# EBI-Metagenomics/deciphon

Hardware: AMD Instinct MI355X
Metric: GCUPS (Viterbi DP cell updates/sec) (higher is better)
Workload: dtype f32

## Files before the change

deciphon_amd/csrc/viterbi_body.h:

```cpp
#pragma once
#include "dcp_types.h"

#ifndef DCP_FN
#error "include a lane_ops_*.h before viterbi_body.h"
#endif

#define DCP_INF (__builtin_inff())

#define DCP_SL(P, t) (((P) + 5 - (t)) % 5)

#ifndef DCP_LAZY_POSITIONS
#define DCP_LAZY_POSITIONS 6
#endif
constexpr int dcp_lazy_turns(int Q) { return Q >= DCP_LAZY_POSITIONS ? 1 : (DCP_LAZY_POSITIONS + Q - 1) / Q; }

#ifndef DCP_SHAPE_POLICY
#define DCP_SHAPE_POLICY(Q, W) ((W) == 1 ? ((Q) > 8 ? 7 : (Q) == 8 ? 2 : 0) : ((Q) >= 8 ? 6 : 0))
#endif
#ifndef DCP_COST_POLICY
#define DCP_COST_POLICY(Q, W) (DCP_SHAPE_POLICY(Q, W) | ((W) == 1 && ((Q) == 4 || (Q) == 5) ? 1 : 0))
#endif
template <int Q, int W, bool STORE = false, int POLICY = DCP_SHAPE_POLICY(Q, W)> struct CostWave
{
  static constexpr int TURNS = dcp_lazy_turns(Q);
  static constexpr bool LATE_FETCH = (POLICY & 1) != 0;
  static constexpr bool STASH = (POLICY & 6) != 0;
  static constexpr bool STASH6 = (POLICY & 4) != 0;
  static constexpr bool CHUNKED = STASH6 && W == 1;
  static constexpr int SLOTS = STASH6 ? 8 : 4;
  Group<W> g;
  float *__restrict__ tab_cells = nullptr;
  float *__restrict__ tab_sp = nullptr;
  int tabKp = 0;
  float *__restrict__ ckpt_out = nullptr;
  float const *__restrict__ ckpt_in = nullptr;
  int ckpt_every = 0;
  int row_base = 0;

  DCP_FN void save_ring(float *__restrict__ to)
  {
#pragma unroll
    for (int s = 0; s < 5; ++s)
    {
      store_q<Q>(to + (size_t)s * tabKp, g.lane, Mpre[s]);
      store_q<Q>(to + (size_t)(5 + s) * tabKp, g.lane, Ipre[s]);
      store_lane(to + (size_t)10 * tabKp + s * 64 * W, g.lane, Spre[s]);
    }
    store_lane(to + (size_t)10 * tabKp + 5 * 64 * W, g.lane, X);
  }
  DCP_FN void load_ring(float const *__restrict__ from)
  {
#pragma unroll
    for (int s = 0; s < 5; ++s)
    {
      load_q<Q>(from + (size_t)s * tabKp, g.lane, Mpre[s]);
      load_q<Q>(from + (size_t)(5 + s) * tabKp, g.lane, Ipre[s]);
      Spre[s] = load_lane(from + (size_t)10 * tabKp + s * 64 * W, g.lane);
    }
    X = load_lane(from + (size_t)10 * tabKp + 5 * 64 * W, g.lane);
  }
  lf BM[Q], MM[Q], MI[Q], MD[Q], IM[Q], II[Q], DM[Q], DD[Q];
  lf Mpre[5][Q], Ipre[5][Q], Spre[5];
  lf em[5][Q];
  lf sa, sb;
  lf X;
  lf NBv, EBv, JBv;
  lf shM, shI, shD;
  float nil[5], bgv[5];
  float ET, CT, RR;
  float E;
  RowSrc rows;
  lu voff;
  uint32_t stride_bytes;
#ifdef DCP_COST_ORDER
  static constexpr bool ORDERED = !STORE && Q >= 5;
  lu voffc[ORDERED ? DcpRowChunks<Q>::N : 1];
#endif
  DcpCodeRow const *__restrict__ codes;

  DcpCodeRow cr;

  DCP_FN void fetch(int l_after, int L)
  {
#pragma unroll
    for (int t = 0; t < 5; ++t)
    {
      uint32_t const off = cr.c[t] * stride_bytes;
#ifdef DCP_COST_ORDER
      if constexpr (ORDERED)
      {
        load_row_hdr(rows, off, nil[t], bgv[t]);
        load_row_chunks<Q>(rows, voffc, off, em[t]);
        continue;
      }
#endif
      load_row_hdr(rows, off, nil[t], bgv[t]);
      load_row_q<Q>(rows, voff, off, em[t]);
    }
    cr = codes[l_after <= L ? l_after : L];
  }

  DCP_FN void init(float const *__restrict__ pool, DcpProfileDev const &pf, DcpCodeRow const *__restrict__ code_rows,
                   float const *__restrict__ xt)
  {
#ifndef DCP_WAVE_PRIO
#define DCP_WAVE_PRIO(Q, W) ((W) > 1 || (Q) >= 6 ? 3 : (Q) >= 4 ? 2 : (Q) == 3 ? 1 : 0)
#endif
    wave_priority<DCP_WAVE_PRIO(Q, W)>();
    g.init();
    lu const lane = g.lane;
    int const Kp = pf.Kp;
    stride_bytes = (uint32_t)(Kp + DCP_ROW_HDR) * 4u;
    int64_t rows_off = pf.rows_off;
#ifdef DCP_COST_ORDER
    if constexpr (ORDERED)
    {
      bool const copy = pf.cost_rows_off != 0 && pf.cost_shape == DCP_COST_SHAPE(Q, W);
      if (copy)
      {
        rows_off = pf.cost_rows_off;
        stride_bytes = 4u * (uint32_t)(DCP_COST_ORDER_HDR + 64 * Q * W);
      }
      row_chunk_offsets<Q, W>(lane, copy, voffc);
    }
#endif
    rows = rowsrc_make(pool + rows_off, (uint32_t)DCP_TABLE_SIZE * stride_bytes);
    voff = row_lane_offset<Q>(lane);
    codes = code_rows;
    float const *__restrict__ trans = pool + pf.trans_off;
    load_q<Q>(trans + DCP_BM * Kp, lane, BM);
    load_q<Q>(trans + DCP_MM * Kp, lane, MM);
    load_q<Q>(trans + DCP_MI * Kp, lane, MI);
    load_q<Q>(trans + DCP_MD * Kp, lane, MD);
    load_q<Q>(trans + DCP_IM * Kp, lane, IM);
    load_q<Q>(trans + DCP_II * Kp, lane, II);
    load_q<Q>(trans + DCP_DM * Kp, lane, DM);
    load_q<Q>(trans + DCP_DD * Kp, lane, DD);
    NBv = lf_pin(xt[DCP_NB]);
    EBv = lf_pin(xt[DCP_EB]);
    JBv = lf_pin(xt[DCP_JB]);
    shM = shI = shD = lf_splat(DCP_INF);
    g.put_tdd(DD);
    if constexpr (STASH)
    {
      g.template stash_q<Q, SLOTS>(0, MD);
      g.template stash_q<Q, SLOTS>(1, DD);
      g.template stash_q<Q, SLOTS>(2, II);
      g.template stash_q<Q, SLOTS>(3, MI);
      if constexpr (STASH6)
      {
        g.template stash_q<Q, SLOTS>(4, IM);
        g.template stash_q<Q, SLOTS>(5, DM);
        g.template stash_q<Q, SLOTS>(6, BM);
        g.template stash_q<Q, SLOTS>(7, MM);
      }
    }
    ET = xt[DCP_ET];
    CT = xt[DCP_CT];
    RR = xt[DCP_RR];
    float const SN = xt[DCP_SN], SB = xt[DCP_SB];
    lm const l0 = lequ(lane, lu_splat(0)), l1 = lequ(lane, lu_splat(1));
    lm const l2 = lequ(lane, lu_splat(2)), l3 = lequ(lane, lu_splat(3));
    lf const inf = lf_splat(DCP_INF);
    sa = lsel(l1, lf_splat(xt[DCP_EJ]), lsel(l2, lf_splat(xt[DCP_EC]), inf));
    sb = lsel(l0, lf_splat(xt[DCP_NN]),
              lsel(l1, lf_splat(xt[DCP_JJ]), lsel(l2, lf_splat(xt[DCP_CC]), lsel(l3, lf_splat(RR), inf))));
#pragma unroll
    for (int s = 0; s < 5; ++s)
    {
      Spre[s] = inf;
#pragma unroll
      for (int q = 0; q < Q; ++q)
      {
        Mpre[s][q] = inf;
        Ipre[s][q] = inf;
      }
    }
#pragma unroll
    for (int q = 0; q < Q; ++q) Mpre[0][q] = lf_splat(SB) + BM[q];
    Spre[0] = lsel(l0, lf_splat(0.0f + SN), lsel(l3, lf_splat(-RR + RR), inf));
    X = lsel(l3, lf_splat(-RR), inf);
    E = DCP_INF;
    tabKp = Kp;
    if (ckpt_in)
      load_ring(ckpt_in);
    else if (STORE)
      store_row0(SB);
  }

  template <int P> DCP_FN void row(int l, int L)
  {
    lf M[Q], I[Q];
#pragma unroll
    for (int q = 0; q < Q; ++q)
    {
      M[q] = lmin3(lmin3(Mpre[DCP_SL(P, 5)][q] + em[4][q], Mpre[DCP_SL(P, 4)][q] + em[3][q],
                         Mpre[DCP_SL(P, 3)][q] + em[2][q]),
                   Mpre[DCP_SL(P, 2)][q] + em[1][q], Mpre[DCP_SL(P, 1)][q] + em[0][q]);
      I[q] = lmin3(lmin3(Ipre[DCP_SL(P, 5)][q] + bgv[4], Ipre[DCP_SL(P, 4)][q] + bgv[3],
                         Ipre[DCP_SL(P, 3)][q] + bgv[2]),
                   Ipre[DCP_SL(P, 2)][q] + bgv[1], Ipre[DCP_SL(P, 1)][q] + bgv[0]);
    }
    X = lmin3(lmin3(Spre[DCP_SL(P, 5)] + nil[4], Spre[DCP_SL(P, 4)] + nil[3], Spre[DCP_SL(P, 3)] + nil[2]),
              Spre[DCP_SL(P, 2)] + nil[1], Spre[DCP_SL(P, 1)] + nil[0]);

    if constexpr (!LATE_FETCH)
      if (l < L) fetch(l + 2, L);

    lf m = M[0];
#pragma unroll
    for (int q = 1; q < Q; ++q) m = lmin(m, M[q]);
    lf D[Q];
    lf Msh0, Ish0, Dsh0, B;
    float N, J;
    if constexpr (STASH)
    {
      g.template unstash_q<Q, SLOTS>(0, MD);
      g.template unstash_q<Q, SLOTS>(1, DD);
    }
    if constexpr (W == 1)
    {
      Msh0 = lane_shift_up_keep(M[Q - 1], shM);
      Ish0 = lane_shift_up_keep(I[Q - 1], shI);
      E = wave_min(m);
      N = read_lane(X, 0);
      J = read_lane(X, 1);
      B = lmin3(N + NBv, E + EBv, J + JBv);

      D[0] = Msh0 + MD[0];
#pragma unroll
      for (int q = 1; q < Q; ++q) D[q] = lmin(M[q - 1] + MD[q], D[q - 1] + DD[q]);
      Dsh0 = lane_shift_up_keep(D[Q - 1], shD);
      lf x = Dsh0 + DD[0];
#pragma unroll
      for (int turn = 0; turn < TURNS; ++turn)
      {
        D[0] = lmin(D[0], x);
#pragma unroll
        for (int q = 1; q < Q; ++q) D[q] = lmin(D[q], D[q - 1] + DD[q]);
        Dsh0 = lane_shift_up_keep(D[Q - 1], shD);
        x = Dsh0 + DD[0];
      }
      while (wave_any(llt(x, D[0])))
      {
        D[0] = lmin(D[0], x);
#pragma unroll
        for (int q = 1; q < Q; ++q) D[q] = lmin(D[q], D[q - 1] + DD[q]);
        Dsh0 = lane_shift_up_keep(D[Q - 1], shD);
        x = Dsh0 + DD[0];
      }
    }
    else
    {
      int const par = l & 1;
      lf const inf = lf_splat(DCP_INF);
      lf x, Dsh;
      lm better;
      D[0] = g.seg_shift_up(M[Q - 1], inf) + MD[0];
#pragma unroll
      for (int q = 1; q < Q; ++q) D[q] = lmin(M[q - 1] + MD[q], D[q - 1] + DD[q]);
      Dsh = g.seg_shift_up(D[Q - 1], inf);
      x = Dsh + DD[0];
      better = llt(x, D[0]);
      while (g.seg_any(better))
      {
        D[0] = lmin(D[0], x);
#pragma unroll
        for (int q = 1; q < Q; ++q) D[q] = lmin(D[q], D[q - 1] + DD[q]);
        Dsh = g.seg_shift_up(D[Q - 1], inf);
        x = Dsh + DD[0];
        better = llt(x, D[0]);
      }
      g.put_rec(par, M[Q - 1], I[Q - 1], D[Q - 1], m);
      g.put_lanes4(GS_X0 + par, X);
      g.sync();
      lf Mp, Ip, Dp;
      bool could;
      g.get_prev(par, Mp, Ip, Dp);
      g.get_e_could(par, E, could);
      g.get_nj(GS_X0 + par, X, N, J);
      Msh0 = g.seg_shift_up(M[Q - 1], Mp);
      Ish0 = g.seg_shift_up(I[Q - 1], Ip);
      B = lmin3(N + NBv, E + EBv, J + JBv);
      if (!could)
      {
        D[0] = lsel(g.seg_first(), lmin(Mp + MD[0], Dp + DD[0]), D[0]);
#pragma unroll
        for (int q = 1; q < Q; ++q) D[q] = lmin(D[q], D[q - 1] + DD[q]);
        Dsh0 = g.seg_shift_up(D[Q - 1], Dp);
        x = Dsh0 + DD[0];
        better = llt(x, D[0]);
        while (g.seg_any(better))
        {
          D[0] = lmin(D[0], x);
#pragma unroll
          for (int q = 1; q < Q; ++q) D[q] = lmin(D[q], D[q - 1] + DD[q]);
          Dsh0 = g.seg_shift_up(D[Q - 1], Dp);
          x = Dsh0 + DD[0];
          better = llt(x, D[0]);
        }
      }
      else
      {
        g.note_fallback();
        D[0] = Msh0 + MD[0];
#pragma unroll
        for (int q = 1; q < Q; ++q) D[q] = lmin(M[q - 1] + MD[q], D[q - 1] + DD[q]);
        g.put_last(GS_D, D[Q - 1]);
        g.sync();
        Dsh0 = g.get_shift(GS_D, D[Q - 1], DCP_INF);
        x = Dsh0 + DD[0];
        better = llt(x, D[0]);
        g.put_any(GS_F, better);
        g.sync();
        while (g.get_any(GS_F, better))
        {
          D[0] = lmin(D[0], x);
#pragma unroll
          for (int q = 1; q < Q; ++q) D[q] = lmin(D[q], D[q - 1] + DD[q]);
          g.put_last(GS_D, D[Q - 1]);
          g.sync();
          Dsh0 = g.get_shift(GS_D, D[Q - 1], DCP_INF);
          x = Dsh0 + DD[0];
          better = llt(x, D[0]);
          g.put_any(GS_F, better);
          g.sync();
        }
      }
    }

    if constexpr (LATE_FETCH)
    {
      sched_fence();
      if (l < L) fetch(l + 2, L);
      sched_fence();
    }
    if constexpr (CHUNKED)
    {
      constexpr int N = DcpStashChunk<Q>::N;
#pragma unroll
      for (int j = 0; j < Q / N; ++j)
      {
        lf bm[N], mm[N], im[N], dm[N], ii[N], mi[N];
        g.template unstash_chunk<Q, SLOTS>(2, j, ii);
        g.template unstash_chunk<Q, SLOTS>(3, j, mi);
        g.template unstash_chunk<Q, SLOTS>(4, j, im);
        g.template unstash_chunk<Q, SLOTS>(5, j, dm);
        g.template unstash_chunk<Q, SLOTS>(6, j, bm);
        g.template unstash_chunk<Q, SLOTS>(7, j, mm);
#pragma unroll
        for (int i = 0; i < N; ++i)
        {
          int const q = N * j + i;
          lf const Ml = q ? M[q ? q - 1 : 0] : Msh0;
          lf const Il = q ? I[q ? q - 1 : 0] : Ish0;
          lf const Dl = q ? D[q ? q - 1 : 0] : Dsh0;
          Mpre[P][q] = lmin3(B + bm[i], Ml + mm[i], lmin(Il + im[i], Dl + dm[i]));
          Ipre[P][q] = lmin(I[q] + ii[i], M[q] + mi[i]);
        }
        sched_fence();
      }
    }
    else if constexpr (STASH)
    {
      g.template unstash_q<Q, SLOTS>(2, II);
      g.template unstash_q<Q, SLOTS>(3, MI);
      if constexpr (STASH6)
      {
        g.template unstash_q<Q, SLOTS>(4, IM);
        g.template unstash_q<Q, SLOTS>(5, DM);
        g.template unstash_q<Q, SLOTS>(6, BM);
        g.template unstash_q<Q, SLOTS>(7, MM);
      }
    }
    if constexpr (!CHUNKED)
    {
#pragma unroll
      for (int q = 0; q < Q; ++q)
      {
        lf const Ml = q ? M[q ? q - 1 : 0] : Msh0;
        lf const Il = q ? I[q ? q - 1 : 0] : Ish0;
        lf const Dl = q ? D[q ? q - 1 : 0] : Dsh0;
        Mpre[P][q] = lmin3(B + BM[q], Ml + MM[q], lmin(Il + IM[q], Dl + DM[q]));
        Ipre[P][q] = lmin(I[q] + II[q], M[q] + MI[q]);
      }
    }
    Spre[P] = lmin(lf_splat(E) + sa, X + sb);
    if (STORE)
    {
      float *row = tab_cells + (size_t)(l - row_base) * 3 * (size_t)tabKp;
      store_q<Q>(row, g.lane, M);
      store_q<Q>(row + tabKp, g.lane, I);
      store_q<Q>(row + 2 * tabKp, g.lane, D);
      float const C = g.get_lane(GS_X0 + (l & 1), X, 2);
      store_sp_lane0(tab_sp + (size_t)(l - row_base) * DCP_SP_STRIDE, g.lane, lf_splat(N), B, lf_splat(J), lf_splat(E),
                     lf_splat(C));
    }
  }

  DCP_FN void store_row0(float SB)
  {
    lf inf[Q];
#pragma unroll
    for (int q = 0; q < Q; ++q) inf[q] = lf_splat(DCP_INF);
    store_q<Q>(tab_cells, g.lane, inf);
    store_q<Q>(tab_cells + tabKp, g.lane, inf);
    store_q<Q>(tab_cells + 2 * tabKp, g.lane, inf);
    lf const i = lf_splat(DCP_INF);
    store_sp_lane0(tab_sp, g.lane, i, lf_splat(SB), i, i, i);
  }

  DCP_FN void run(int L, float *out, int Lend = -1)
  {
    if (Lend < 0 || Lend > L) Lend = L;
    int l = row_base + 1;
    if (l <= Lend)
    {
      cr = codes[l];
      fetch(l + 1, Lend);
    }
    for (; l + 4 <= Lend; l += 5)
    {
      row<1>(l, Lend);
      row<2>(l + 1, Lend);
      row<3>(l + 2, Lend);
      row<4>(l + 3, Lend);
      row<0>(l + 4, Lend);
      if (ckpt_every > 0 && (l + 4) % ckpt_every == 0 && l + 4 + 5 < L)
        save_ring(ckpt_out + (size_t)((l + 4) / ckpt_every - 1) * (size_t)dcp_ckpt_floats(tabKp, W));
    }
    if (l <= Lend) row<1>(l++, Lend);
    if (l <= Lend) row<2>(l++, Lend);
    if (l <= Lend) row<3>(l++, Lend);
    if (l <= Lend) row<4>(l++, Lend);
    if (Lend < L) return;
    g.sync();
    g.put_lanes4(GS_X, X);
    g.sync();
    float const C = g.get_lane(GS_X, X, 2);
    float const R = g.get_lane(GS_X, X, 3);
    float const T = L > 0 ? __builtin_fminf(E + ET, C + CT) : DCP_INF;
    store_f32_lane0(out + 0, g.lane, R);
    store_f32_lane0(out + 1, g.lane, T);
  }
};

template <int Q, int W, bool STORE = false> struct StripWave
{
  Group<W> g;
  float *__restrict__ tab_cells = nullptr;
  float *__restrict__ tab_sp = nullptr;
  float *__restrict__ ring = nullptr;
  float const *__restrict__ trans = nullptr;
  int Kp = 0, S = 0;
  lf Spre[5];
  lf sa, sb, X;
  float Bz[5];
  float NB, EB, JB, ET, CT, RR, E;
  RowSrc rows;
  lu voff;
  uint32_t stride_bytes;
  DcpCodeRow const *__restrict__ codes;
  int tick = 0;
  float *__restrict__ ckpt_out = nullptr;
  float const *__restrict__ ckpt_in = nullptr;
  int ckpt_every = 0;
  int row_base = 0;

  enum { KS = 64 * Q * W };

  DCP_FN void save_ring(float *__restrict__ to)
  {
    for (int s = 0; s < S; ++s)
      for (int z = 0; z < 10; ++z)
      {
        lf v[Q];
        load_q<Q>(ring + (size_t)z * Kp + (size_t)s * KS, g.lane, v);
        store_q<Q>(to + (size_t)z * Kp + (size_t)s * KS, g.lane, v);
      }
    float *sp = to + (size_t)10 * Kp;
#pragma unroll
    for (int z = 0; z < 5; ++z)
    {
      store_lane(sp + z * 64 * W, g.lane, Spre[z]);
      store_f32_lane0(sp + DCP_CKPT_SP * 64 * W + z, g.lane, Bz[z]);
    }
    store_lane(sp + 5 * 64 * W, g.lane, X);
  }
  DCP_FN void load_ring(float const *__restrict__ from)
  {
    for (int s = 0; s < S; ++s)
      for (int z = 0; z < 10; ++z)
      {
        lf v[Q];
        load_q<Q>(from + (size_t)z * Kp + (size_t)s * KS, g.lane, v);
        store_q<Q>(ring + (size_t)z * Kp + (size_t)s * KS, g.lane, v);
      }
    float const *sp = from + (size_t)10 * Kp;
#pragma unroll
    for (int z = 0; z < 5; ++z)
    {
      Spre[z] = load_lane(sp + z * 64 * W, g.lane);
      Bz[z] = sp[DCP_CKPT_SP * 64 * W + z];
    }
    X = load_lane(sp + 5 * 64 * W, g.lane);
  }

  DCP_FN void init(float const *__restrict__ pool, DcpProfileDev const &pf, DcpCodeRow const *__restrict__ code_rows,
                   float const *__restrict__ xt)
  {
    g.init();
    lu const lane = g.lane;
    Kp = pf.Kp;
    S = Kp / KS;
    stride_bytes = (uint32_t)(Kp + DCP_ROW_HDR) * 4u;
    rows = rowsrc_make(pool + pf.rows_off, (uint32_t)DCP_TABLE_SIZE * stride_bytes);
    voff = row_lane_offset<Q>(lane);
    codes = code_rows;
    trans = pool + pf.trans_off;
    NB = xt[DCP_NB];
    EB = xt[DCP_EB];
    JB = xt[DCP_JB];
    ET = xt[DCP_ET];
    CT = xt[DCP_CT];
    RR = xt[DCP_RR];
    float const SN = xt[DCP_SN], SB = xt[DCP_SB];
    lm const l0 = lequ(lane, lu_splat(0)), l1 = lequ(lane, lu_splat(1));
    lm const l2 = lequ(lane, lu_splat(2)), l3 = lequ(lane, lu_splat(3));
    lf const inf = lf_splat(DCP_INF);
    sa = lsel(l1, lf_splat(xt[DCP_EJ]), lsel(l2, lf_splat(xt[DCP_EC]), inf));
    sb = lsel(l0, lf_splat(xt[DCP_NN]),
              lsel(l1, lf_splat(xt[DCP_JJ]), lsel(l2, lf_splat(xt[DCP_CC]), lsel(l3, lf_splat(RR), inf))));
#pragma unroll
    for (int z = 0; z < 5; ++z)
    {
      Spre[z] = inf;
      Bz[z] = DCP_INF;
    }
    Bz[0] = SB;
    Spre[0] = lsel(l0, lf_splat(0.0f + SN), lsel(l3, lf_splat(-RR + RR), inf));
    X = lsel(l3, lf_splat(-RR), inf);
    E = DCP_INF;
    lf infq[Q];
#pragma unroll
    for (int q = 0; q < Q; ++q) infq[q] = inf;
    for (int s = 0; s < S; ++s)
    {
      lf DD[Q];
      load_q<Q>(trans + (size_t)DCP_DD * Kp + (size_t)s * KS, lane, DD);
      g.put_tdd_strip(s, DD);
      if (ckpt_in) continue;
      for (int z = 0; z < 10; ++z) store_q<Q>(ring + (size_t)z * Kp + (size_t)s * KS, lane, infq);
      if (STORE)
        for (int z = 0; z < 3; ++z) store_q<Q>(tab_cells + (size_t)z * Kp + (size_t)s * KS, lane, infq);
    }
    if (ckpt_in)
      load_ring(ckpt_in);
    else if (STORE)
      store_sp_lane0(tab_sp, lane, inf, lf_splat(SB), inf, inf, inf);
    g.put_carry_inf(0);
    g.put_carry_inf(1);
    g.sync();
  }

  template <int P> DCP_FN void row(int l)
  {
    lu const lane = g.lane;
    lf const inf = lf_splat(DCP_INF);
    DcpCodeRow const cr = codes[l];
    uint32_t off[5];
    float nil[5], bgv[5];
#pragma unroll
    for (int t = 0; t < 5; ++t)
    {
      off[t] = cr.c[t] * stride_bytes;
      load_row_hdr(rows, off[t], nil[t], bgv[t]);
    }
    X = lmin3(lmin3(Spre[DCP_SL(P, 5)] + nil[4], Spre[DCP_SL(P, 4)] + nil[3], Spre[DCP_SL(P, 3)] + nil[2]),
              Spre[DCP_SL(P, 2)] + nil[1], Spre[DCP_SL(P, 1)] + nil[0]);
    g.put_lanes4(GS_X0 + (l & 1), X);
    float Erun = DCP_INF;
    for (int s = 0; s < S; ++s)
    {
      size_t const col = (size_t)s * KS;
      lf BM[Q], MM[Q], MI[Q], MD[Q], IM[Q], II[Q], DM[Q], DD[Q];
      load_q<Q>(trans + (size_t)DCP_BM * Kp + col, lane, BM);
      load_q<Q>(trans + (size_t)DCP_MM * Kp + col, lane, MM);
      load_q<Q>(trans + (size_t)DCP_MI * Kp + col, lane, MI);
      load_q<Q>(trans + (size_t)DCP_MD * Kp + col, lane, MD);
      load_q<Q>(trans + (size_t)DCP_IM * Kp + col, lane, IM);
      load_q<Q>(trans + (size_t)DCP_II * Kp + col, lane, II);
      load_q<Q>(trans + (size_t)DCP_DM * Kp + col, lane, DM);
      load_q<Q>(trans + (size_t)DCP_DD * Kp + col, lane, DD);
      lf M[Q], I[Q], D[Q];
#pragma unroll
      for (int q = 0; q < Q; ++q) M[q] = I[q] = inf;
#pragma unroll
      for (int t = 5; t >= 1; --t)
      {
        lf r[Q], ip[Q], em[Q];
        load_q<Q>(ring + (size_t)DCP_SL(P, t) * Kp + col, lane, r);
        load_q<Q>(ring + (size_t)(5 + DCP_SL(P, t)) * Kp + col, lane, ip);
        load_row_q<Q>(rows, voff + (uint32_t)(col * 4), off[t - 1], em);
#pragma unroll
        for (int q = 0; q < Q; ++q)
        {
          M[q] = lmin(M[q], lmin(Bz[DCP_SL(P, t)] + BM[q], r[q]) + em[q]);
          I[q] = lmin(I[q], ip[q] + bgv[t - 1]);
        }
      }
      lf m = M[0];
#pragma unroll
      for (int q = 1; q < Q; ++q) m = lmin(m, M[q]);

      int const par = tick;
      tick ^= 1;
      lf x, Dsh;
      lm better;
      D[0] = g.seg_shift_up(M[Q - 1], inf) + MD[0];
#pragma unroll
      for (int q = 1; q < Q; ++q) D[q] = lmin(M[q - 1] + MD[q], D[q - 1] + DD[q]);
      Dsh = g.seg_shift_up(D[Q - 1], inf);
      x = Dsh + DD[0];
      better = llt(x, D[0]);
      while (g.seg_any(better))
      {
        D[0] = lmin(D[0], x);
#pragma unroll
        for (int q = 1; q < Q; ++q) D[q] = lmin(D[q], D[q - 1] + DD[q]);
        Dsh = g.seg_shift_up(D[Q - 1], inf);
        x = Dsh + DD[0];
        better = llt(x, D[0]);
      }
      g.put_rec(par, M[Q - 1], I[Q - 1], D[Q - 1], m);
      g.sync();
      lf Mp, Ip, Dp;
      float Es;
      bool could;
      g.get_prev(par, Mp, Ip, Dp);
      g.get_e_could_row(par, s, Erun, Es, could);
      lf const Msh0 = g.seg_shift_up(M[Q - 1], Mp);
      lf const Ish0 = g.seg_shift_up(I[Q - 1], Ip);
      lf Dsh0;
      if (!could)
      {
        D[0] = lsel(g.seg_first(), lmin(Mp + MD[0], Dp + DD[0]), D[0]);
#pragma unroll
        for (int q = 1; q < Q; ++q) D[q] = lmin(D[q], D[q - 1] + DD[q]);
        Dsh0 = g.seg_shift_up(D[Q - 1], Dp);
        x = Dsh0 + DD[0];
        better = llt(x, D[0]);
        while (g.seg_any(better))
        {
          D[0] = lmin(D[0], x);
#pragma unroll
          for (int q = 1; q < Q; ++q) D[q] = lmin(D[q], D[q - 1] + DD[q]);
          Dsh0 = g.seg_shift_up(D[Q - 1], Dp);
          x = Dsh0 + DD[0];
          better = llt(x, D[0]);
        }
      }
      else
      {
        g.note_fallback();
        D[0] = Msh0 + MD[0];
#pragma unroll
        for (int q = 1; q < Q; ++q) D[q] = lmin(M[q - 1] + MD[q], D[q - 1] + DD[q]);
        g.put_last(GS_D, D[Q - 1]);
        g.sync();
        Dsh0 = g.get_shift_carry(GS_D, D[Q - 1], Dp);
        x = Dsh0 + DD[0];
        better = llt(x, D[0]);
        g.put_any(GS_F, better);
        g.sync();
        while (g.get_any(GS_F, better))
        {
          D[0] = lmin(D[0], x);
#pragma unroll
          for (int q = 1; q < Q; ++q) D[q] = lmin(D[q], D[q - 1] + DD[q]);
          g.put_last(GS_D, D[Q - 1]);
          g.sync();
          Dsh0 = g.get_shift_carry(GS_D, D[Q - 1], Dp);
          x = Dsh0 + DD[0];
          better = llt(x, D[0]);
          g.put_any(GS_F, better);
          g.sync();
        }
      }
      Erun = __builtin_fminf(Erun, Es);

      lf rest[Q], ipre[Q];
#pragma unroll
      for (int q = 0; q < Q; ++q)
      {
        lf const Ml = q ? M[q ? q - 1 : 0] : Msh0;
        lf const Il = q ? I[q ? q - 1 : 0] : Ish0;
        lf const Dl = q ? D[q ? q - 1 : 0] : Dsh0;
        rest[q] = lmin3(Ml + MM[q], Il + IM[q], Dl + DM[q]);
        ipre[q] = lmin(I[q] + II[q], M[q] + MI[q]);
      }
      store_q<Q>(ring + (size_t)P * Kp + col, lane, rest);
      store_q<Q>(ring + (size_t)(5 + P) * Kp + col, lane, ipre);
      if (STORE)
      {
        float *trow = tab_cells + (size_t)(l - row_base) * 3 * (size_t)Kp + col;
        store_q<Q>(trow, lane, M);
        store_q<Q>(trow + Kp, lane, I);
        store_q<Q>(trow + 2 * (size_t)Kp, lane, D);
      }
      if (s + 1 < S)
        g.put_carry(tick, M[Q - 1], I[Q - 1], D[Q - 1]);
      else
        g.put_carry_inf(tick);
    }
    E = Erun;
    float N, J;
    g.get_nj(GS_X0 + (l & 1), X, N, J);
    float const B = __builtin_fminf(__builtin_fminf(N + NB, E + EB), J + JB);
    Bz[P] = B;
    Spre[P] = lmin(lf_splat(E) + sa, X + sb);
    if (STORE)
    {
      float const C = g.get_lane(GS_X0 + (l & 1), X, 2);
      store_sp_lane0(tab_sp + (size_t)(l - row_base) * DCP_SP_STRIDE, lane, lf_splat(N), lf_splat(B), lf_splat(J), lf_splat(E),
                     lf_splat(C));
    }
  }

  DCP_FN void run(int L, float *out, int Lend = -1)
  {
    if (Lend < 0 || Lend > L) Lend = L;
    int l = row_base + 1;
    for (; l + 4 <= Lend; l += 5)
    {
      row<1>(l);
      row<2>(l + 1);
      row<3>(l + 2);
      row<4>(l + 3);
      row<0>(l + 4);
      if (ckpt_every > 0 && (l + 4) % ckpt_every == 0 && l + 4 + 5 < L)
        save_ring(ckpt_out + (size_t)((l + 4) / ckpt_every - 1) * (size_t)dcp_strip_ckpt_floats(Kp, W));
    }
    if (l <= Lend) row<1>(l++);
    if (l <= Lend) row<2>(l++);
    if (l <= Lend) row<3>(l++);
    if (l <= Lend) row<4>(l++);
    if (Lend < L) return;
    g.sync();
    g.put_lanes4(GS_X, X);
    g.sync();
    float const C = g.get_lane(GS_X, X, 2);
    float const R = g.get_lane(GS_X, X, 3);
    float const T = L > 0 ? __builtin_fminf(E + ET, C + CT) : DCP_INF;
    store_f32_lane0(out + 0, g.lane, R);
    store_f32_lane0(out + 1, g.lane, T);
  }
};

#define DCP_UPD(cur, ptr, val, newptr)                                         \
  do                                                                           \
  {                                                                            \
    lf const v_ = (val);                                                       \
    (ptr) = lselu(llt(v_, (cur)), lu_splat(newptr), (ptr));                    \
    (cur) = lmin((cur), v_);                                                   \
  } while (0)

#define DCP_UPDS(cur, ptr, val, newptr)                                        \
  do                                                                           \
  {                                                                            \
    float const v_ = (val);                                                    \
    if (v_ < (cur)) (ptr) = (newptr);                                          \
    (cur) = __builtin_fminf((cur), v_);                                        \
  } while (0)

template <int Q, int W> struct PathWave
{
  Group<W> g;
  lf BM[Q], MM[Q], MI[Q], MD[Q], IM[Q], II[Q], DM[Q], DD[Q];
  lf M[5][Q], I[5][Q], D[5][Q], Msh[5], Ish[5], Dsh[5];
  float S[5], N[5], B[5], J[5], E[5], C[5];
  float xt[DCP_NUM_XTRANS];
  int K;
  RowSrc rows;
  lu voff;
  uint32_t stride_bytes;
  DcpCodeRow const *__restrict__ codes;
  DcpCodeRow cr;
  lf em[5][Q];
  float nil[5], bgv[5];
  uint32_t *__restrict__ xnodes;
  uint16_t *__restrict__ nodes;

  DCP_FN void init(float const *__restrict__ pool, DcpProfileDev const &pf, DcpCodeRow const *__restrict__ code_rows,
                   float const *__restrict__ xtp, uint32_t *__restrict__ xn, uint16_t *__restrict__ nd)
  {
    g.init();
    lu const lane = g.lane;
    K = pf.K;
    int const Kp = pf.Kp;
    stride_bytes = (uint32_t)(Kp + DCP_ROW_HDR) * 4u;
    rows = rowsrc_make(pool + pf.rows_off, (uint32_t)DCP_TABLE_SIZE * stride_bytes);
    voff = row_lane_offset<Q>(lane);
    codes = code_rows;
    xnodes = xn;
    nodes = nd;
    float const *__restrict__ trans = pool + pf.trans_off;
    load_q<Q>(trans + DCP_BM * Kp, lane, BM);
    load_q<Q>(trans + DCP_MM * Kp, lane, MM);
    load_q<Q>(trans + DCP_MI * Kp, lane, MI);
    load_q<Q>(trans + DCP_MD * Kp, lane, MD);
    load_q<Q>(trans + DCP_IM * Kp, lane, IM);
    load_q<Q>(trans + DCP_II * Kp, lane, II);
    load_q<Q>(trans + DCP_DM * Kp, lane, DM);
    load_q<Q>(trans + DCP_DD * Kp, lane, DD);
#pragma unroll
    for (int i = 0; i < DCP_NUM_XTRANS; ++i) xt[i] = xtp[i];
    lf const inf = lf_splat(DCP_INF);
#pragma unroll
    for (int s = 0; s < 5; ++s)
    {
      S[s] = N[s] = B[s] = J[s] = E[s] = C[s] = DCP_INF;
      Msh[s] = Ish[s] = Dsh[s] = inf;
#pragma unroll
      for (int q = 0; q < Q; ++q) M[s][q] = I[s][q] = D[s][q] = inf;
    }
    S[0] = 0.0f;
    B[0] = xt[DCP_SB];
    store_u32_lane0(xnodes, lane, 0u);
    lu zero[Q];
#pragma unroll
    for (int q = 0; q < Q; ++q) zero[q] = lu_splat(0);
    store_nodes_q<Q>(nodes, K, lane, zero);
  }

  DCP_FN uint32_t e_field(float v, lf const (&Ma)[Q], lf const (&Da)[Q], lf const (&Mbefore)[Q],
                          lf const (&Dbefore)[Q])
  {
    if (!(v < DCP_INF)) return 0u;
    lu const lane = g.lane;
    lf const vv = lf_splat(v);
    lu field = lu_splat(0xffffffffu);
    lm has = llt_u(lu_splat(1), lu_splat(0));
    lm multi = has;
#pragma unroll
    for (int q = 0; q < Q; ++q)
    {
      lu const k2 = (lane * (uint32_t)Q + (uint32_t)q) * 2u;
      lm const mM = leq(Ma[q], vv), mD = leq(Da[q], vv);
      multi = lor(multi, lor(land(has, lor(mM, mD)), land(mM, mD)));
      has = lor(has, lor(mM, mD));
      field = lselu(mD, lminu(field, k2 + 1u), field);
      field = lselu(mM, lminu(field, k2), field);
    }
    g.put_count(GS_F, has);
    g.put_any(GS_X, multi);
    g.put_minu(GS_T0, field);
    g.sync();
    bool const single = g.get_count(GS_F, has) == 1 && !g.get_any(GS_X, multi);
    uint32_t const first = g.get_minu(GS_T0, field);
    if (single) return first;

    int Qr = (K - 1) / DCP_REF_LANES + 1;
    if (Qr < 2) Qr = 2;
    lf stale[Q];
    g.put_last(GS_M, Mbefore[Q - 1]);
    g.sync();
    lf const Mb0 = g.get_shift(GS_M, Mbefore[Q - 1], DCP_INF);
#pragma unroll
    for (int q = 0; q < Q; ++q)
    {
      lf const lastMb = q ? Mbefore[q ? q - 1 : 0] : Mb0;
      stale[q] = lmin(Dbefore[q], lastMb + MD[q]);
    }
    uint32_t best = 0;
    for (int er = 0; er < DCP_REF_LANES; ++er)
    {
      lu ord = lu_splat(0xffffffffu);
#pragma unroll
      for (int q = 0; q < Q; ++q)
      {
        lu const k = lane * (uint32_t)Q + (uint32_t)q;
        lu const lo = lu_splat((uint32_t)(er * Qr));
        lm const in = land(lnot(llt_u(k, lo)), llt_u(k, lo + (uint32_t)Qr));
        lu const qr = k - lo;
        lu const ordM = qr * 2u;
        lu const ordD = lselu(lequ(qr, lu_splat(0)),
                              lselu(leq(stale[q], vv), lu_splat(1u), lu_splat((uint32_t)(2 * Qr))), qr * 2u + 1u);
        ord = lselu(land(in, leq(Ma[q], vv)), lminu(ord, ordM), ord);
        ord = lselu(land(in, leq(Da[q], vv)), lminu(ord, ordD), ord);
      }
      int const slot = (er & 1) ? GS_T1 : GS_T0;
      g.put_minu(slot, ord);
      g.sync();
      uint32_t const w = g.get_minu(slot, ord);
      if (w != 0xffffffffu)
      {
        uint32_t name, qr;
        if (w == (uint32_t)(2 * Qr)) { name = 2u; qr = 0u; }
        else { name = (w & 1u) ? 2u : 1u; qr = w >> 1; }
        uint32_t const packed = (name << 28) | ((uint32_t)er << 24) | qr;
        if (packed > best) best = packed;
      }
    }
    uint32_t const q = best & 0x00ffffffu, e = (best >> 24) & 0xfu;
    uint32_t const k = e * (uint32_t)Qr + q;
    return 2u * k + ((best >> 28) == 2u ? 1u : 0u);
  }

  template <int T, int Z>
  DCP_FN void pass(int l, lf (&Ma)[Q], lf (&Ia)[Q], lf (&Da)[Q], lu (&pM)[Q], lu (&pI)[Q], lu (&pD)[Q], float &Na,
                   float &Ba, float &Ja, float &Ea, float &Ca, float &Ta, uint32_t &pN, uint32_t &pB, uint32_t &pJ,
                   uint32_t &pE, uint32_t &pC, uint32_t &pT)
  {
    (void)l;
    constexpr uint32_t u = (uint32_t)(T - 1);
    float const nil = this->nil[T - 1];
    float const bg = this->bgv[T - 1];
    lf const(&em)[Q] = this->em[T - 1];

    DCP_UPDS(Na, pN, (S[Z] + xt[DCP_SN]) + nil, 0u + u);
    DCP_UPDS(Na, pN, (N[Z] + xt[DCP_NN]) + nil, 5u + u);
    DCP_UPDS(Ba, pB, Na + xt[DCP_NB], 1u);
    DCP_UPDS(Ja, pJ, (E[Z] + xt[DCP_EJ]) + nil, 0u + u);
    DCP_UPDS(Ja, pJ, (J[Z] + xt[DCP_JJ]) + nil, 5u + u);
    DCP_UPDS(Ca, pC, (E[Z] + xt[DCP_EC]) + nil, 0u + u);
    DCP_UPDS(Ca, pC, (C[Z] + xt[DCP_CC]) + nil, 5u + u);

    lf Mbefore[Q], Dbefore[Q];
#pragma unroll
    for (int q = 0; q < Q; ++q)
    {
      Mbefore[q] = Ma[q];
      Dbefore[q] = Da[q];
    }

    lf const Bz = lf_splat(B[Z]);
#pragma unroll
    for (int q = 0; q < Q; ++q)
    {
      lf const Ml = q ? M[Z][q ? q - 1 : 0] : Msh[Z];
      lf const Il = q ? I[Z][q ? q - 1 : 0] : Ish[Z];
      lf const Dl = q ? D[Z][q ? q - 1 : 0] : Dsh[Z];
      DCP_UPD(Ma[q], pM[q], (Bz + BM[q]) + em[q], 0u + u);
      DCP_UPD(Ma[q], pM[q], (Ml + MM[q]) + em[q], 5u + u);
      DCP_UPD(Ma[q], pM[q], (Il + IM[q]) + em[q], 10u + u);
      DCP_UPD(Ma[q], pM[q], (Dl + DM[q]) + em[q], 15u + u);
      DCP_UPD(Ia[q], pI[q], (I[Z][q] + II[q]) + lf_splat(bg), 5u + u);
      DCP_UPD(Ia[q], pI[q], (M[Z][q] + MI[q]) + lf_splat(bg), 0u + u);
    }
    g.put_last(GS_M, Ma[Q - 1]);
    g.sync();
    lf const Mash0 = g.get_shift(GS_M, Ma[Q - 1], DCP_INF);
#pragma unroll
    for (int q = 0; q < Q; ++q)
    {
      lf const lastMa = q ? Ma[q ? q - 1 : 0] : Mash0;
      DCP_UPD(Da[q], pD[q], lastMa + MD[q], 0u);
    }

    lf m = lmin(Ma[0], Da[0]);
#pragma unroll
    for (int q = 1; q < Q; ++q) m = lmin(m, lmin(Ma[q], Da[q]));
    g.put_min(GS_E, m);
    g.sync();
    Ea = g.get_min(GS_E, m);
    if (T == 1) pE = e_field(Ea, Ma, Da, Mbefore, Dbefore);

#pragma unroll
    for (int q = 1; q < Q; ++q) DCP_UPD(Da[q], pD[q], Da[q - 1] + DD[q], 1u);
    for (;;)
    {
      g.put_last(GS_D, Da[Q - 1]);
      g.sync();
      lf const x = g.get_shift(GS_D, Da[Q - 1], DCP_INF) + DD[0];
      lm const better = llt(x, Da[0]);
      g.put_any(GS_F, better);
      g.sync();
      if (!g.get_any(GS_F, better)) break;
      DCP_UPD(Da[0], pD[0], x, 1u);
#pragma unroll
      for (int q = 1; q < Q; ++q) DCP_UPD(Da[q], pD[q], Da[q - 1] + DD[q], 1u);
    }

    DCP_UPDS(Ba, pB, Ea + xt[DCP_EB], 2u);
    DCP_UPDS(Ba, pB, Ja + xt[DCP_JB], 3u);
    DCP_UPDS(Ta, pT, Ea + xt[DCP_ET], 0u);
    DCP_UPDS(Ta, pT, Ca + xt[DCP_CT], 1u);
  }

  DCP_FN void fetch(int l_after, int L)
  {
#pragma unroll
    for (int t = 0; t < 5; ++t)
    {
      uint32_t const off = cr.c[t] * stride_bytes;
      load_row_hdr(rows, off, nil[t], bgv[t]);
      load_row_q<Q>(rows, voff, off, em[t]);
    }
    cr = codes[l_after <= L ? l_after : L];
  }

  template <int P> DCP_FN float row(int l, int L)
  {
    lf const inf = lf_splat(DCP_INF);
    lf Ma[Q], Ia[Q], Da[Q];
    lu pM[Q], pI[Q], pD[Q];
#pragma unroll
    for (int q = 0; q < Q; ++q)
    {
      Ma[q] = Ia[q] = Da[q] = inf;
      pM[q] = pI[q] = pD[q] = lu_splat(0);
    }
    float Na = DCP_INF, Ba = DCP_INF, Ja = DCP_INF, Ea = DCP_INF, Ca = DCP_INF, Ta = DCP_INF;
    uint32_t pN = 0, pB = 0, pJ = 0, pE = 0, pC = 0, pT = 0;

    if (l >= 5) pass<5, DCP_SL(P, 5)>(l, Ma, Ia, Da, pM, pI, pD, Na, Ba, Ja, Ea, Ca, Ta, pN, pB, pJ, pE, pC, pT);
    if (l >= 4) pass<4, DCP_SL(P, 4)>(l, Ma, Ia, Da, pM, pI, pD, Na, Ba, Ja, Ea, Ca, Ta, pN, pB, pJ, pE, pC, pT);
    if (l >= 3) pass<3, DCP_SL(P, 3)>(l, Ma, Ia, Da, pM, pI, pD, Na, Ba, Ja, Ea, Ca, Ta, pN, pB, pJ, pE, pC, pT);
    if (l >= 2) pass<2, DCP_SL(P, 2)>(l, Ma, Ia, Da, pM, pI, pD, Na, Ba, Ja, Ea, Ca, Ta, pN, pB, pJ, pE, pC, pT);
    pass<1, DCP_SL(P, 1)>(l, Ma, Ia, Da, pM, pI, pD, Na, Ba, Ja, Ea, Ca, Ta, pN, pB, pJ, pE, pC, pT);
    if (l < L) fetch(l + 2, L);

    lu const lane = g.lane;
    store_u32_lane0(xnodes + l, lane, (pN << 0) | (pB << 4) | (pE << 6) | (pC << 21) | (pT << 25) | (pJ << 26));
    lu w[Q];
#pragma unroll
    for (int q = 0; q < Q; ++q)
    {
      lu const k = lane * (uint32_t)Q + (uint32_t)q;
      lu word = pM[q];
      word = word | lselu(lequ(k, lu_splat(0)), lu_splat(0), pD[q] << 5);
      word = word | lselu(llt_u(k + 1u, lu_splat((uint32_t)K)), pI[q] << 6, lu_splat(0));
      w[q] = word;
    }
    store_nodes_q<Q>(nodes + (size_t)l * (size_t)K, K, lane, w);

#pragma unroll
    for (int q = 0; q < Q; ++q)
    {
      M[P][q] = Ma[q];
      I[P][q] = Ia[q];
      D[P][q] = Da[q];
    }
    g.put_last(GS_M, Ma[Q - 1]);
    g.put_last(GS_I, Ia[Q - 1]);
    g.put_last(GS_D, Da[Q - 1]);
    g.sync();
    Msh[P] = g.get_shift(GS_M, Ma[Q - 1], DCP_INF);
    Ish[P] = g.get_shift(GS_I, Ia[Q - 1], DCP_INF);
    Dsh[P] = g.get_shift(GS_D, Da[Q - 1], DCP_INF);
    S[P] = DCP_INF;
    N[P] = Na;
    B[P] = Ba;
    J[P] = Ja;
    E[P] = Ea;
    C[P] = Ca;
    return Ta;
  }

  DCP_FN float run(int L)
  {
    float T = DCP_INF;
    if (L > 0)
    {
      cr = codes[1];
      fetch(2, L);
    }
    int l = 1;
    for (; l + 4 <= L; l += 5)
    {
      T = row<1>(l, L);
      T = row<2>(l + 1, L);
      T = row<3>(l + 2, L);
      T = row<4>(l + 3, L);
      T = row<0>(l + 4, L);
    }
    if (l <= L) T = row<1>(l++, L);
    if (l <= L) T = row<2>(l++, L);
    if (l <= L) T = row<3>(l++, L);
    if (l <= L) T = row<4>(l++, L);
    return T;
  }
};
```

deciphon_amd/csrc/viterbi_pack.h:

```cpp
#pragma once
#include "dcp_types.h"

#ifndef DCP_FN
#error "include a lane_ops_*.h before viterbi_pack.h"
#endif

#ifndef DCP_INF
#error "include viterbi_body.h before viterbi_pack.h"
#endif
#ifndef DCP_SL
#define DCP_SL(P, t) (((P) + 5 - (t)) % 5)
#endif

#define DCP_PACK_LDS_ROW(Q, S) ((DCP_ROW_HDR + ((S)-1) * (Q) + 3) / 4 * 4)
#define DCP_PACK_LDS_ROWS(NLDS) ((NLDS) == 5 ? 1364 : (NLDS) == 4 ? 340 : (NLDS) == 3 ? 84 : (NLDS) == 2 ? 20 : 4)

#ifndef DCP_PACK_LATE
#define DCP_PACK_LATE(Q) ((Q) == 4)
#endif
template <int Q, int S, int TURNS = dcp_lazy_turns(Q), int NLDS = 0, bool LATE = DCP_PACK_LATE(Q)> struct PackWave
{
  static constexpr bool LDSTAB = NLDS > 0;
  static_assert(S == 4 || S == 8 || S == 16 || S == 32, "groups of 4, 8, 16 or 32 lanes");
  enum { G = 64 / S, CAP = (S - 1) * Q };
#ifndef DCP_PACK_STASH
#define DCP_PACK_STASH 1
#endif
  static constexpr bool STASH = DCP_PACK_STASH && Q >= 3 && Q <= 4;
  lf MD[Q], DD[Q];
  lf Mpre[5][Q], Ipre[5][Q], Spre[5];
  enum { EQ = Q < 2 ? 2 : Q };
  lf em[5][EQ];
  lu code[5];
  lf sa, sb, nbjb;
  lf X, E;
  lf EBv;
  lf shM, shI, shD;
  lf Xs, Es;
  lu Lg;
  lu crow;
  PackSrc src;
  lds_float const *lds_rows = nullptr;
  lu lds_off;

  lf kBM[STASH ? 1 : Q], kMM[STASH ? 1 : Q], kIM[STASH ? 1 : Q], kDM[STASH ? 1 : Q], kII[STASH ? 1 : Q], kMI[STASH ? 1 : Q];
  DCP_FN void set_fold_trans(lf const (&BM)[Q], lf const (&MM)[Q], lf const (&IM)[Q], lf const (&DM)[Q],
                             lf const (&II)[Q], lf const (&MI)[Q])
  {
    if constexpr (STASH)
    {
      pack_stash<Q>(0, BM);
      pack_stash<Q>(1, MM);
      pack_stash<Q>(2, IM);
      pack_stash<Q>(3, DM);
      pack_stash<Q>(4, II);
      pack_stash<Q>(5, MI);
    }
    else
    {
#pragma unroll
      for (int q = 0; q < Q; ++q)
      {
        kBM[q] = BM[q];
        kMM[q] = MM[q];
        kIM[q] = IM[q];
        kDM[q] = DM[q];
        kII[q] = II[q];
        kMI[q] = MI[q];
      }
    }
  }
  DCP_FN void get_fold_trans(PackFold &f, lf (&BM)[Q], lf (&MM)[Q], lf (&IM)[Q], lf (&DM)[Q], lf (&II)[Q], lf (&MI)[Q])
  {
    if constexpr (STASH)
      pack_unstash_wait<Q>(f, BM, MM, IM, DM, II, MI);
    else
    {
#pragma unroll
      for (int q = 0; q < Q; ++q)
      {
        BM[q] = kBM[q];
        MM[q] = kMM[q];
        IM[q] = kIM[q];
        DM[q] = kDM[q];
        II[q] = kII[q];
        MI[q] = kMI[q];
      }
    }
  }

  DCP_FN void fetch_codes(int l) { load_code_row(src, crow + (uint32_t)l, code); }

  DCP_FN void fetch_rows()
  {
#pragma unroll
    for (int t = 0; t < 5; ++t)
    {
      if (t < NLDS)
        load_lds_q<EQ>(lds_rows, code[t] * (uint32_t)DCP_PACK_LDS_ROW(Q, S) + lds_off, em[t]);
      else
        load_pack_q<EQ>(src, code[t], em[t]);
    }
  }

  DCP_FN void init(float const *__restrict__ pool, DcpProfileDev const &pf, DcpCodeRow const *__restrict__ code_rows,
                   uint32_t ncode_rows, float const *__restrict__ xt_table, DcpPack const &pk,
                   lds_float const *lds_table = nullptr)
  {
    lds_rows = lds_table;
    lu const lane = lane_ids();
    lu const e = lane & lu_splat((uint32_t)(S - 1));
    lu const g = lane_shr(lane, S == 4 ? 2 : S == 8 ? 3 : S == 16 ? 4 : 5);
    int const Kp = pf.Kp;
    lm const sep = lequ(e, lu_splat(0));
    lu const col = lselu(sep, lu_splat((uint32_t)(Kp - Q)), (e - lu_splat(1)) * (uint32_t)Q);
    src = packsrc_make(pool + pf.rows_off, Kp, code_rows, ncode_rows,
                       lselu(sep, lu_splat(0), (col + (uint32_t)DCP_ROW_HDR) * 4u));
    lds_off = lselu(sep, lu_splat(0), col + (uint32_t)DCP_ROW_HDR);
    float const *__restrict__ trans = pool + pf.trans_off;
    lf BM[Q], MM[Q], MI[Q], IM[Q], II[Q], DM[Q];
    load_cols<Q>(trans + DCP_BM * Kp, col, BM);
    load_cols<Q>(trans + DCP_MM * Kp, col, MM);
    load_cols<Q>(trans + DCP_MI * Kp, col, MI);
    load_cols<Q>(trans + DCP_MD * Kp, col, MD);
    load_cols<Q>(trans + DCP_IM * Kp, col, IM);
    load_cols<Q>(trans + DCP_II * Kp, col, II);
    load_cols<Q>(trans + DCP_DM * Kp, col, DM);
    load_cols<Q>(trans + DCP_DD * Kp, col, DD);
    set_fold_trans(BM, MM, IM, DM, II, MI);
    Lg = load_u32_at(reinterpret_cast<uint32_t const *>(pk.L), g);
    crow = load_u32_at(pk.code_row, g);
    lu const xrow = load_u32_at(reinterpret_cast<uint32_t const *>(pk.xt_row), g) * (uint32_t)DCP_XT_STRIDE;
    lf const inf = lf_splat(DCP_INF);
    lm const l0 = lequ(e, lu_splat(0)), l1 = lequ(e, lu_splat(1)), l2 = lequ(e, lu_splat(2)), l3 = lequ(e, lu_splat(3));
    lf const NB = load_f32_at(xt_table, xrow + (uint32_t)DCP_NB), JB = load_f32_at(xt_table, xrow + (uint32_t)DCP_JB);
    lf const RR = load_f32_at(xt_table, xrow + (uint32_t)DCP_RR), SN = load_f32_at(xt_table, xrow + (uint32_t)DCP_SN);
    lf const SB = load_f32_at(xt_table, xrow + (uint32_t)DCP_SB);
    EBv = load_f32_at(xt_table, xrow + (uint32_t)DCP_EB);
    sa = lsel(l1, load_f32_at(xt_table, xrow + (uint32_t)DCP_EJ), lsel(l2, load_f32_at(xt_table, xrow + (uint32_t)DCP_EC), inf));
    sb = lsel(l0, load_f32_at(xt_table, xrow + (uint32_t)DCP_NN),
              lsel(l1, load_f32_at(xt_table, xrow + (uint32_t)DCP_JJ),
                   lsel(l2, load_f32_at(xt_table, xrow + (uint32_t)DCP_CC), lsel(l3, RR, inf))));
    nbjb = lsel(l0, NB, lsel(l1, JB, inf));
    shM = shI = shD = inf;
#pragma unroll
    for (int s = 0; s < 5; ++s)
    {
      Spre[s] = inf;
#pragma unroll
      for (int q = 0; q < Q; ++q)
      {
        Mpre[s][q] = inf;
        Ipre[s][q] = inf;
      }
    }
#pragma unroll
    for (int q = 0; q < Q; ++q) Mpre[0][q] = SB + BM[q];
    Spre[0] = lsel(l0, lf_splat(0.0f) + SN, lsel(l3, lneg(RR) + RR, inf));
    X = lsel(l3, lneg(RR), inf);
    E = inf;
    Xs = X;
    Es = inf;
  }

  template <int P> DCP_FN void row(int l, int Lmax)
  {
    lf M[Q], I[Q], D[Q];
    lf bgv[5], hdr[5], sp[5], xs[5];
#pragma unroll
    for (int t = 0; t < 5; ++t)
    {
      bgv[t] = group_bcast0<S>(em[t][1]);
      hdr[t] = em[t][0];
      sp[t] = Spre[DCP_SL(P, t + 1)];
    }
    add_quad0_x5(xs, sp, hdr);
#pragma unroll
    for (int q = 0; q < Q; ++q)
    {
      M[q] = lmin3(lmin3(Mpre[DCP_SL(P, 5)][q] + em[4][q], Mpre[DCP_SL(P, 4)][q] + em[3][q],
                         Mpre[DCP_SL(P, 3)][q] + em[2][q]),
                   Mpre[DCP_SL(P, 2)][q] + em[1][q], Mpre[DCP_SL(P, 1)][q] + em[0][q]);
      I[q] = lmin3(lmin3(Ipre[DCP_SL(P, 5)][q] + bgv[4], Ipre[DCP_SL(P, 4)][q] + bgv[3],
                         Ipre[DCP_SL(P, 3)][q] + bgv[2]),
                   Ipre[DCP_SL(P, 2)][q] + bgv[1], Ipre[DCP_SL(P, 1)][q] + bgv[0]);
    }
    X = lmin3(lmin3(xs[4], xs[3], xs[2]), xs[1], xs[0]);

    if constexpr (!LATE)
    {
      if (l < Lmax)
      {
        fetch_rows();
        fetch_codes(l + 2);
      }
    }

    lf m = M[0];
#pragma unroll
    for (int q = 1; q < Q; ++q) m = lmin(m, M[q]);
    lf const Msh0 = lane_shift_up_keep(M[Q - 1], shM);
    lf const Ish0 = lane_shift_up_keep(I[Q - 1], shI);
    E = group_min<S>(m);
    lf const B = lmin(E + EBv, group_min01<S>(X + nbjb));

    PackFold fold;
    if constexpr (STASH) pack_unstash_issue(fold);

    D[0] = Msh0 + MD[0];
#pragma unroll
    for (int q = 1; q < Q; ++q) D[q] = lmin(M[q - 1] + MD[q], D[q - 1] + DD[q]);
    lf Dsh0 = lane_shift_up_keep(D[Q - 1], shD);
    lf x = Dsh0 + DD[0];
#pragma unroll
    for (int turn = 0; turn < TURNS; ++turn)
    {
      D[0] = lmin(D[0], x);
#pragma unroll
      for (int q = 1; q < Q; ++q) D[q] = lmin(D[q], D[q - 1] + DD[q]);
      Dsh0 = lane_shift_up_keep(D[Q - 1], shD);
      x = Dsh0 + DD[0];
    }
    while (wave_any(llt(x, D[0])))
    {
      D[0] = lmin(D[0], x);
#pragma unroll
      for (int q = 1; q < Q; ++q) D[q] = lmin(D[q], D[q - 1] + DD[q]);
      Dsh0 = lane_shift_up_keep(D[Q - 1], shD);
      x = Dsh0 + DD[0];
    }

    if constexpr (LATE)
    {
      sched_fence();
      if (l < Lmax)
      {
        fetch_rows();
        fetch_codes(l + 2);
      }
      sched_fence();
    }
    lf BM[Q], MM[Q], IM[Q], DM[Q], II[Q], MI[Q];
    get_fold_trans(fold, BM, MM, IM, DM, II, MI);
#pragma unroll
    for (int q = 0; q < Q; ++q)
    {
      lf const Ml = q ? M[q ? q - 1 : 0] : Msh0;
      lf const Il = q ? I[q ? q - 1 : 0] : Ish0;
      lf const Dl = q ? D[q ? q - 1 : 0] : Dsh0;
      Mpre[P][q] = lmin3(B + BM[q], Ml + MM[q], lmin(Il + IM[q], Dl + DM[q]));
      Ipre[P][q] = lmin(I[q] + II[q], M[q] + MI[q]);
    }
    Spre[P] = lmin(E + sa, X + sb);
    lm const last = lequ(Lg, lu_splat((uint32_t)l));
    Xs = lsel(last, X, Xs);
    Es = lsel(last, E, Es);
  }

  DCP_FN void run(int Lmax, float *__restrict__ out, DcpPack const &pk, float const *__restrict__ xt_table)
  {
    if (Lmax > 0)
    {
      fetch_codes(1);
      fetch_rows();
      fetch_codes(2);
    }
    int l = 1;
    for (; l + 4 <= Lmax; l += 5)
    {
      row<1>(l, Lmax);
      row<2>(l + 1, Lmax);
      row<3>(l + 2, Lmax);
      row<4>(l + 3, Lmax);
      row<0>(l + 4, Lmax);
    }
    if (l <= Lmax) row<1>(l++, Lmax);
    if (l <= Lmax) row<2>(l++, Lmax);
    if (l <= Lmax) row<3>(l++, Lmax);
    if (l <= Lmax) row<4>(l++, Lmax);
    lu const lane = lane_ids();
    lu const e = lane & lu_splat((uint32_t)(S - 1));
    lu const g = lane_shr(lane, S == 4 ? 2 : S == 8 ? 3 : S == 16 ? 4 : 5);
    lu const slot = load_u32_at(reinterpret_cast<uint32_t const *>(pk.out), g);
    lu const xrow = load_u32_at(reinterpret_cast<uint32_t const *>(pk.xt_row), g) * (uint32_t)DCP_XT_STRIDE;
    lm const active = llt_u(lu_splat(0), Lg);
    lf const T = lmin(Es + load_f32_at(xt_table, xrow + (uint32_t)DCP_ET), Xs + load_f32_at(xt_table, xrow + (uint32_t)DCP_CT));
    store_f32_where(out, slot * 2u + 1u, land(active, lequ(e, lu_splat(2))), T);
    store_f32_where(out, slot * 2u, land(active, lequ(e, lu_splat(3))), Xs);
  }
};
```

Before: 840.6.

## Propagate lazy-F delete carry as scalar chain, apply to D vector once

Replaces the striped lazy-F delete fix-up loops with a helper that propagates only the carry value across lanes. It uses a running sum of the DD transitions instead of rewriting every D[q] on each turn, and applies the min to the full D vector once at the end. This cuts the per-turn work from Q mins plus adds to a chain of adds and one min, which shortens the dependency chain around the cross-lane shifts. Correctness relies on the min-plus carry composing the same way as the element-wise updates; the extra adds may change float rounding slightly.

```diff
diff --git a/deciphon_amd/csrc/viterbi_body.h b/deciphon_amd/csrc/viterbi_body.h
--- a/deciphon_amd/csrc/viterbi_body.h
+++ b/deciphon_amd/csrc/viterbi_body.h
@@ -13,6 +13,56 @@
 #define DCP_LAZY_POSITIONS 6
 #endif
 constexpr int dcp_lazy_turns(int Q) { return Q >= DCP_LAZY_POSITIONS ? 1 : (DCP_LAZY_POSITIONS + Q - 1) / Q; }
+
+template <int Q, int TURNS> DCP_FN lf dcp_lazy_turns_carry(lf (&D)[Q], lf const (&DD)[Q], lf &shD)
+{
+  lf c = lane_shift_up_keep(D[Q - 1], shD);
+#pragma unroll
+  for (int turn = 1; turn < TURNS; ++turn)
+  {
+    lf r = c + DD[0];
+#pragma unroll
+    for (int q = 1; q < Q; ++q) r = r + DD[q];
+    c = lane_shift_up_keep(lmin(D[Q - 1], r), shD);
+  }
+  if constexpr (TURNS > 0)
+  {
+    lf r = c + DD[0];
+    D[0] = lmin(D[0], r);
+#pragma unroll
+    for (int q = 1; q < Q; ++q)
+    {
+      r = r + DD[q];
+      D[q] = lmin(D[q], r);
+    }
+    c = lane_shift_up_keep(D[Q - 1], shD);
+  }
+  lf x = c + DD[0];
+  if (wave_any(llt(x, D[0])))
+  {
+    lf d0 = D[0], last = D[Q - 1], applied;
+    do
+    {
+      applied = c;
+      d0 = lmin(d0, x);
+      lf r = x;
+#pragma unroll
+      for (int q = 1; q < Q; ++q) r = r + DD[q];
+      last = Q > 1 ? lmin(last, r) : d0;
+      c = lane_shift_up_keep(last, shD);
+      x = c + DD[0];
+    } while (wave_any(llt(x, d0)));
+    lf r = applied + DD[0];
+    D[0] = lmin(D[0], r);
+#pragma unroll
+    for (int q = 1; q < Q; ++q)
+    {
+      r = r + DD[q];
+      D[q] = lmin(D[q], r);
+    }
+  }
+  return c;
+}
 
 #ifndef DCP_SHAPE_POLICY
 #define DCP_SHAPE_POLICY(Q, W) ((W) == 1 ? ((Q) > 8 ? 7 : (Q) == 8 ? 2 : 0) : ((Q) >= 8 ? 6 : 0))
@@ -230,25 +280,7 @@
       D[0] = Msh0 + MD[0];
 #pragma unroll
       for (int q = 1; q < Q; ++q) D[q] = lmin(M[q - 1] + MD[q], D[q - 1] + DD[q]);
-      Dsh0 = lane_shift_up_keep(D[Q - 1], shD);
-      lf x = Dsh0 + DD[0];
-#pragma unroll
-      for (int turn = 0; turn < TURNS; ++turn)
-      {
-        D[0] = lmin(D[0], x);
-#pragma unroll
-        for (int q = 1; q < Q; ++q) D[q] = lmin(D[q], D[q - 1] + DD[q]);
-        Dsh0 = lane_shift_up_keep(D[Q - 1], shD);
-        x = Dsh0 + DD[0];
-      }
-      while (wave_any(llt(x, D[0])))
-      {
-        D[0] = lmin(D[0], x);
-#pragma unroll
-        for (int q = 1; q < Q; ++q) D[q] = lmin(D[q], D[q - 1] + DD[q]);
-        Dsh0 = lane_shift_up_keep(D[Q - 1], shD);
-        x = Dsh0 + DD[0];
-      }
+      Dsh0 = dcp_lazy_turns_carry<Q, TURNS>(D, DD, shD);
     }
     else
     {
diff --git a/deciphon_amd/csrc/viterbi_pack.h b/deciphon_amd/csrc/viterbi_pack.h
--- a/deciphon_amd/csrc/viterbi_pack.h
+++ b/deciphon_amd/csrc/viterbi_pack.h
@@ -210,25 +210,7 @@
     D[0] = Msh0 + MD[0];
 #pragma unroll
     for (int q = 1; q < Q; ++q) D[q] = lmin(M[q - 1] + MD[q], D[q - 1] + DD[q]);
-    lf Dsh0 = lane_shift_up_keep(D[Q - 1], shD);
-    lf x = Dsh0 + DD[0];
-#pragma unroll
-    for (int turn = 0; turn < TURNS; ++turn)
-    {
-      D[0] = lmin(D[0], x);
-#pragma unroll
-      for (int q = 1; q < Q; ++q) D[q] = lmin(D[q], D[q - 1] + DD[q]);
-      Dsh0 = lane_shift_up_keep(D[Q - 1], shD);
-      x = Dsh0 + DD[0];
-    }
-    while (wave_any(llt(x, D[0])))
-    {
-      D[0] = lmin(D[0], x);
-#pragma unroll
-      for (int q = 1; q < Q; ++q) D[q] = lmin(D[q], D[q - 1] + DD[q]);
-      Dsh0 = lane_shift_up_keep(D[Q - 1], shD);
-      x = Dsh0 + DD[0];
-    }
+    lf const Dsh0 = dcp_lazy_turns_carry<Q, TURNS>(D, DD, shD);
 
     if constexpr (LATE)
     {
```

Measured after the change: 865.7 (median of 6 runs). 1.03x the previous value.
